# RetamalVictor/marl-range-flocking

Measured on AMD Instinct MI355X. Metric: agent-steps/sec at 256 agents x 4096 envs; 1/2/4/8 MI355X, higher is better.
Workload: dtype f32; 1 GPU; gym_flock_v2 step, 256 agents x 4096 envs per GPU (BASELINE config 3); agents=256, envs_per_gpu=4096, k=4, periodic=True, parallelism=env-shard x1

## Files before the change

marl_range_flocking_amd/csrc/flock_env.hip:

```cpp
#include <hip/hip_runtime.h>

#include <stdint.h>
#include <stdio.h>
#include <stdlib.h>
#include <string.h>

#include "flock_amd.h"
#include "flock_mem.h"

#pragma clang fp contract(off)

namespace {

constexpr int kMem = 4;
constexpr int kSense = 4;
constexpr float kHalfPi = 1.57079637f;
constexpr uint32_t kEmpty = 0xFFFFFFFFu;

thread_local char g_err[256] = "";

int fail(int code, const char* msg) {
    snprintf(g_err, sizeof(g_err), "%s", msg);
    return code;
}
// ... 1747 lines not shown
        FLOCK_CASE(5)
        FLOCK_CASE(6)
        FLOCK_CASE(7)
        FLOCK_CASE(8)
        FLOCK_CASE(9)
        FLOCK_CASE(10)
        FLOCK_CASE(11)
        FLOCK_CASE(12)
        FLOCK_CASE(17)
        default:
            return fail(FLOCK_E_LIMIT, "unsupported k");
    }
#undef FLOCK_CASE
    const hipError_t e = hipGetLastError();
    if (e != hipSuccess) return fail(FLOCK_E_LAUNCH, hipGetErrorString(e));
    return FLOCK_OK;
}

Params base(int E, int N, int k, float box) {
    Params p;
    memset(&p, 0, sizeof(p));
    p.E = E;
    p.N = N;
    p.k = k;
    p.box = box;
    p.clamp = 1;
    return p;
}

}


void flock_sc_diag_no_spec(bool v);
void flock_sc_diag_event_system(bool v);
void flock_sc_diag_free_events(bool v);

extern "C" {

int flock_abi_version(void) { return FLOCK_ABI_VERSION; }

int flock_set_diag(const char* name, int value) {
    if (!name) return fail(FLOCK_E_NULL, "flock_set_diag: NULL name");
    Knobs& k = knobs_mut();
    if (!strcmp(name, "env_launches"))
        k.env_launches = value;
    else if (!strcmp(name, "no_spec"))
        k.no_spec = value != 0;
    else if (!strcmp(name, "no_split"))
        k.no_split = value != 0;
    else if (!strcmp(name, "no_cells"))
        k.no_cells = value != 0;
    else if (!strcmp(name, "pf"))
        k.pf = value;
    else if (!strcmp(name, "rollout_spl") && (value == 2 || value == 4))
        k.rollout_spl = value;
    else if (!strcmp(name, "sc_no_spec"))
        flock_sc_diag_no_spec(value != 0);
    else if (!strcmp(name, "sc_event_system_scope"))
        flock_sc_diag_event_system(value != 0);
    else if (!strcmp(name, "sc_free_events"))
        flock_sc_diag_free_events(value != 0);
    else
        return fail(FLOCK_E_ARG, "flock_set_diag: unknown knob");
    return FLOCK_OK;
}

#ifdef FLOCK_PHASE_PROF
int flock_phase_read(unsigned long long* host) {
    static unsigned long long buf[64 * 32];
    if (hipMemcpyFromSymbol(buf, HIP_SYMBOL(g_phase), sizeof(buf)) != hipSuccess) return 1;
    for (int q = 0; q < 32; ++q) {
        host[q] = 0;
        for (int s = 0; s < 64; ++s) host[q] += buf[s * 32 + q];
    }
    memset(buf, 0, sizeof(buf));
    return hipMemcpyToSymbol(HIP_SYMBOL(g_phase), buf, sizeof(buf)) != hipSuccess;
}
int flock_blk_read(unsigned long long* host) {
    return hipMemcpyFromSymbol(host, HIP_SYMBOL(g_blk), sizeof(g_blk)) != hipSuccess;
}
int flock_blkph_read(unsigned long long* host) {
    return hipMemcpyFromSymbol(host, HIP_SYMBOL(g_blkph), sizeof(g_blkph)) != hipSuccess;
}
#endif

const char* flock_last_error(void) { return g_err; }

}

namespace {
// ... 400 lines not shown
```

marl_range_flocking_amd/csrc/flock_sc.hip:

```cpp
#include <hip/hip_runtime.h>

#include <math.h>
#include <stdint.h>
#include <stdlib.h>

#include "flock_learn.h"
#include "flock_mem.h"
#include "learn_internal.h"

namespace {

using flock_learn_internal::fail;
using flock_learn_internal::launched;

constexpr int kRowsPerBlock = 4;
constexpr int kMaxAct = 4;
constexpr int kMaxIn = 64;
constexpr int kMaxFeat = 1024;
constexpr int kMaxFc1Block = 32768;
constexpr float kLnEps = 1e-5f;

typedef float f32x16 __attribute__((ext_vector_type(16)));

struct CriticOff {
// ... 537 lines not shown
            for (int o = 0; o < kMaxAct; ++o)
                if (o < na) dh = fmaf(aWmu[o * H2 + j], dm[o], dh);
            g2[c] = ag2[j];
        }
        dy2[c] = h2[c] > 0.0f ? dh : 0.0f;
    }
    ln_backward<C>(dy2, xh, g2, rs, H2, dz2);
    store_row<C>(w.AXH2 + ro, xh, H2, lane);
    store_row<C>(w.AH2 + ro, h2, H2, lane);
    store_row<C>(w.ADY2 + ro, dy2, H2, lane);
    store_row<C>(w.ADZ2 + ro, dz2, H2, lane);
    if (lane == 0) w.ARS2[r] = rs;
}

#ifdef FLOCK_SC_PROF
__device__ unsigned long long g_scprof[5][4096][2];
struct ScProf {
    int k;
    unsigned long long t0;
    __device__ explicit ScProf(int kk) : k(kk), t0(__builtin_amdgcn_s_memrealtime()) {}
    __device__ ~ScProf() {
        const int b = blockIdx.x + gridDim.x * blockIdx.y;
        if (b < 4096 && (threadIdx.x & 63) == 0) {
            if (threadIdx.x == 0) g_scprof[k][b][0] = t0;
            atomicMax(&g_scprof[k][b][1], (unsigned long long)__builtin_amdgcn_s_memrealtime());
        }
    }
};
#define SC_PROF(k) ScProf sc_prof_(k)
__device__ unsigned long long g_scmark[4096][8];
#define SC_MARK(MK, i)                                                                           \
    if (MK && threadIdx.x == 0 && blockIdx.x + gridDim.x * blockIdx.y < 4096)                   \
        g_scmark[blockIdx.x + gridDim.x * blockIdx.y][i] = __builtin_amdgcn_s_memrealtime();
#else
#define SC_PROF(k)
#define SC_MARK(MK, i)
#endif
#ifdef FLOCK_SC_PRIO
#define SC_WAVE_PRIO() __builtin_amdgcn_s_setprio(FLOCK_SC_PRIO)
#else
#define SC_WAVE_PRIO()
#endif
constexpr unsigned long long kGateTimeoutTicks = 200000000ull;
__device__ __forceinline__ bool gate_wait(unsigned long long* gate, unsigned long long seq,
                                          unsigned long long* err = nullptr,
                                          unsigned long long ticks = kGateTimeoutTicks) {
    __shared__ int ok;
    if (threadIdx.x == 0) {
        int good = 1;
        if ((long long)(flock_mem::ld_sc1(gate) - seq) < 0) {
            const unsigned long long t0 = __builtin_amdgcn_s_memrealtime();
            while ((long long)(flock_mem::ld_sc1(gate) - seq) < 0) {
                if (__builtin_amdgcn_s_memrealtime() - t0 > ticks) {
                    __hip_atomic_store(err ? err : gate + 1, 1ull, __ATOMIC_RELAXED, __HIP_MEMORY_SCOPE_AGENT);
                    good = 0;
                    break;
                }
                __builtin_amdgcn_s_sleep(2);
            }
        }
        ok = good;
    }
    __syncthreads();
    return ok != 0;
}

__device__ __forceinline__ int xcd_perm(int x, int n) { return (n & 7) == 0 ? (x & 7) * (n >> 3) + (x >> 3) : x; }

template <int C, int HC>
// ... 284 lines not shown
    for (int q = 0; q < 4; ++q) {
        const int m = tm * kT + 8 * wv + 4 * (l >> 5) + q;
        if (m < g.M && n < g.N) g.C[(int64_t)m * g.ldc + n] = g.bias ? out[q] + bias : out[q];
    }
}

template <int AV, int BV, int NF>
__global__ __launch_bounds__(256) void sc_gemm(GemmBatch gb) {
    SC_PROF(1);
    SC_WAVE_PRIO();
    if (gb.done && blockIdx.x == 0 && blockIdx.y == 0 && threadIdx.x == 0) flock_mem::st_sc1(gb.done, gb.done_seq);
    gemm_block<AV, BV, NF>(gb, blockIdx.y, blockIdx.x);
}

struct RedP {
    const float* D;
    const float* X;
    int ldd, ldx, mode, in, n, blk0;
    int64_t off;
};
constexpr int kMaxRed = 12;
#ifndef FLOCK_RED_RB
#define FLOCK_RED_RB 8
#endif
constexpr int kRedElems = 16;
constexpr int kRedGroups = 256 / kRedElems;
constexpr int kMaxRedBlocks = 4096;

struct DzArgs {
    const float *XH, *RS, *PS;
    int F, ntn;
};

__device__ __forceinline__ float red_block(const RedP& rp, int b, int B, const DzArgs& dz, float* part, float* mst,
                                           int& e_out, bool& live_out) {
    const int tid = threadIdx.x;
    const bool dzm = rp.mode == 4 || rp.mode == 5;
    const int el = tid & (kRedElems - 1), q = tid / kRedElems;
    const int e = (b - rp.blk0) * kRedElems + el;
    const bool live = e < rp.n;
    const bool per_in = rp.mode == 2 || rp.mode == 4;
    const int o = per_in ? e / rp.in : e;
    const int i = per_in ? e - o * rp.in : e;
    const bool prod = rp.mode == 1 || rp.mode == 2 || rp.mode == 4;
    constexpr int kRB = FLOCK_RED_RB;
    float dv[kRB], xv[kRB], xh[kRB], rs[kRB];
    auto load = [&](int r0) {
#pragma unroll
        for (int k = 0; k < kRB; ++k) {
            const int r = r0 + kRedGroups * k;
            const bool in = live && r < B;
            dv[k] = in ? rp.D[(int64_t)r * rp.ldd + o] : 0.0f;
            xv[k] = (in && prod) ? rp.X[(int64_t)r * rp.ldx + i] : 0.0f;
            xh[k] = (in && dzm) ? dz.XH[(int64_t)r * dz.F + o] : 0.0f;
            rs[k] = (in && dzm) ? dz.RS[r] : 0.0f;
        }
    };
    load(q);
    if (dzm) {
        for (int r = tid; r < B; r += 256) {
            const float2* ps = reinterpret_cast<const float2*>(dz.PS + (int64_t)r * 2 * dz.ntn);
            float s1 = 0.0f, s2 = 0.0f;
            constexpr int kPB = 16;
            for (int t0 = 0; t0 < dz.ntn; t0 += kPB) {
                float2 v[kPB];
#pragma unroll
                for (int u = 0; u < kPB; ++u)
                    v[u] = t0 + u < dz.ntn ? ps[t0 + u] : make_float2(0.0f, 0.0f);
#pragma unroll
                for (int u = 0; u < kPB; ++u)
                    if (t0 + u < dz.ntn) {
                        s1 += v[u].x;
                        s2 += v[u].y;
                    }
            }
            mst[2 * r] = s1 / (float)dz.F;
            mst[2 * r + 1] = s2 / (float)dz.F;
        }
        __syncthreads();
    }
    float acc = 0.0f;
    for (int r0 = q; r0 < B; r0 += kRedGroups * kRB) {
        if (r0 != q) load(r0);
        if (dzm) {
#pragma unroll
            for (int k = 0; k < kRB; ++k) {
                const int r = min(r0 + kRedGroups * k, B - 1);
                dv[k] = rs[k] * (dv[k] - mst[2 * r] - xh[k] * mst[2 * r + 1]);
            }
        }
#pragma unroll
        for (int k = 0; k < kRB; ++k) acc = prod ? fmaf(dv[k], xv[k], acc) : acc + dv[k];
    }
    part[q * kRedElems + el] = acc;
    __syncthreads();
    float gsum = 0.0f;
    if (q == 0 && live) {
#pragma unroll
        for (int k = 0; k < kRedGroups; ++k) gsum += part[k * kRedElems + el];
    }
    e_out = e;
    live_out = live && q == 0;
    return gsum;
}

struct BwdJob {
    GemmP dh;
    GemmP dw;
    const float *H1, *XH1, *g1;
    float *DY1, *DXH1, *PS1;
    int F, ntn;
    int64_t w2_off;
    int nred, nblk, B;
    RedP red[kMaxRed];
    float* grad;
    int64_t rel;
    int64_t grad_rel;
    const int64_t* agent;
    int64_t agent_v;
    float* loss;
};
__host__ __device__ inline int bwd_blocks(const BwdJob& j) { return j.dh.tiles + j.dw.tiles + j.nblk; }

template <int AVH, int BVH, int AVW, int BVW, int NFH, int NFW>
__device__ __forceinline__ void bwd_body(const BwdJob& j, int bx) {
    extern __shared__ float4 smem4[];
// ... 15 lines not shown
            const int m = tm * kT + 8 * wv + 4 * (l >> 5) + q;
            const bool ok = m < g.M && nok;
            hv[q] = ok ? j.H1[(int64_t)m * j.F + n] : 0.0f;
            xv[q] = ok ? j.XH1[(int64_t)m * j.F + n] : 0.0f;
        }
        float out[4];
        gemm_tile<AVH, BVH, NFH>(g, g.B + relB, tm, tn, smem, out);
        float s1[4], s2[4];
#pragma unroll
        for (int q = 0; q < 4; ++q) {
            const int m = tm * kT + 8 * wv + 4 * (l >> 5) + q;
            const bool ok = m < g.M && nok;
            const float dy = hv[q] > 0.0f ? out[q] : 0.0f;
            const float dxh = dy * gam;
            if (ok) {
                j.DY1[(int64_t)m * j.F + n] = dy;
                j.DXH1[(int64_t)m * j.F + n] = dxh;
            }
            s1[q] = ok ? dxh : 0.0f;
            s2[q] = ok ? dxh * xv[q] : 0.0f;
        }
#pragma unroll
        for (int off = 16; off >= 1; off >>= 1)
#pragma unroll
            for (int q = 0; q < 4; ++q) {
                s1[q] += __shfl_xor(s1[q], off);
                s2[q] += __shfl_xor(s2[q], off);
            }
        if ((l & 31) == 0) {
#pragma unroll
            for (int q = 0; q < 4; ++q) {
                const int m = tm * kT + 8 * wv + 4 * (l >> 5) + q;
                if (m < g.M) {
                    j.PS1[((int64_t)m * j.ntn + tn) * 2] = s1[q];
                    j.PS1[((int64_t)m * j.ntn + tn) * 2 + 1] = s2[q];
                }
            }
        }
    } else if (bx < j.dh.tiles + j.dw.tiles) {
        const GemmP& g = j.dw;
        const int t = bx - j.dh.tiles;
        const int tm = t / g.tiles_n, tn = t - tm * g.tiles_n;
        float out[4];
        gemm_tile<AVW, BVW, NFW>(g, g.B, tm, tn, smem, out);
        const int nn = tn * kT + (l & 31);
#pragma unroll
        for (int q = 0; q < 4; ++q) {
            const int mm = tm * kT + 8 * wv + 4 * (l >> 5) + q;
            if (mm < g.M && nn < g.N) j.grad[gbase + j.w2_off + (int64_t)mm * g.ldc + nn] = out[q];
        }
    } else {
        const int b = bx - j.dh.tiles - j.dw.tiles;
        int q0 = 0;
        for (int q = 1; q < j.nred; ++q)
            if (b >= j.red[q].blk0) q0 = q;
        const RedP& rp = j.red[q0];
        int e;
        bool wr;
        const DzArgs none{nullptr, nullptr, nullptr, 0, 0};
        const float gsum = red_block(rp, b, j.B, none, smem, nullptr, e, wr);
        if (wr) {
            if (rp.mode == 3)
                *j.loss = gsum * (1.0f / (float)j.B);
            else
                j.grad[gbase + rp.off + e] = gsum;
        }
    }
}

struct Bwd2 {
    BwdJob j0, j1;
    int nb0;
    int n0;
};
template <int AVH, int BVH, int AVW, int BVW, int NFH, int NFW>
__global__ __launch_bounds__(256) void sc_bwd(Bwd2 bb) {
    SC_PROF(3);
    SC_WAVE_PRIO();
    if ((int)blockIdx.x < bb.nb0) {
        if ((int)blockIdx.x < bb.n0) bwd_body<AVH, BVH, AVW, BVW, NFH, NFW>(bb.j0, blockIdx.x);
    } else {
        bwd_body<AVH, BVH, AVW, BVW, NFH, NFW>(bb.j1, blockIdx.x - bb.nb0);
    }
}

struct GradAdam {
    int nred, nblk, B, do_adam;
    RedP red[kMaxRed];
    DzArgs dz;
    int64_t adam_lo, adam_n;
    int adam_blocks;
    float *p, *grad, *m, *v;
    int64_t rel;
    int64_t grad_rel;
    const float* grad_scale;
    const int64_t* agent;
    int64_t agent_v;
    int64_t* step;
    unsigned* counter;
    float lr, b1, b2, eps;
    float* target;
    float* self_soft;
    int64_t self_n;
    int soft_rate, soft_blocks;
    float tau, one_minus_tau;
    float* p_copy;
    const int64_t* soft_count;
};
__host__ __device__ inline int late_blocks(const GradAdam& ga) { return ga.nblk + ga.adam_blocks + ga.soft_blocks; }

struct AdamState {
    float p, m, v, t;
};
__device__ __forceinline__ AdamState adam_load(const GradAdam& ga, int64_t i) {
    return {ga.p[i], ga.m[i], ga.v[i], ga.target ? ga.target[i] : 0.0f};
}
__device__ __forceinline__ void adam_store(const GradAdam& ga, int64_t i, AdamState s, float gi, float neg_step,
                                           float bc2s, bool soft) {
    const float w1 = (float)(1.0 - (double)ga.b1), omb2 = (float)(1.0 - (double)ga.b2);
    float mi = s.m;
    mi = (w1 < 0.5f) ? mi + w1 * (gi - mi) : gi - (gi - mi) * (1.0f - w1);
    float vi = s.v * ga.b2;
    vi = vi + (omb2 * gi) * gi;
    const float denom = __builtin_sqrtf(vi) / bc2s + ga.eps;
    const float pn = s.p + (neg_step * mi) / denom;
    if (ga.p_copy) {
        ga.p_copy[i] = pn;
        ga.p[i] = soft ? ga.tau * pn + ga.one_minus_tau * pn : pn;
    } else {
        ga.p[i] = pn;
    }
    ga.m[i] = mi;
    ga.v[i] = vi;
    if (soft && ga.target) ga.target[i] = ga.tau * pn + ga.one_minus_tau * s.t;
}

__device__ __forceinline__ void grad_adam_body(const GradAdam& ga, int bx, int nb) {
    extern __shared__ float4 smem4[];
    float* smem = reinterpret_cast<float*>(smem4);
    __shared__ float sh[2];
    __shared__ int sh_soft;
    const int tid = threadIdx.x;
    const int64_t agent = ga.rel ? agent_at(ga.agent, ga.agent_v) : 0;
    const int64_t base = ga.rel * agent, gbase = ga.grad_rel * agent;
    if (tid == 0) {
        const int64_t step0 = ga.do_adam ? ga.step[agent] : 0;
        const int64_t count = ga.soft_count ? ga.soft_count[agent_at(ga.agent, ga.agent_v)] : step0;
        sh_soft = ga.do_adam && ga.soft_rate > 0 && (count % ga.soft_rate) == 0;
        if (ga.do_adam) {
            const double st = (double)(step0 + 1);
            sh[0] = (float)(-(double)ga.lr / (1.0 - pow((double)ga.b1, st)));
            sh[1] = (float)sqrt(1.0 - pow((double)ga.b2, st));
        }
    }
    const int adam0 = ga.nblk, soft0 = ga.nblk + ga.adam_blocks;
    if (bx >= soft0) {
        __syncthreads();
        if (sh_soft && ga.self_soft) {
            const int64_t b0 = (int64_t)(bx - soft0) * 1024;
#pragma unroll
            for (int q = 0; q < 4; ++q) {
                const int64_t e = b0 + q * 256 + tid;
                if (e < ga.self_n) {
                    const float c = ga.self_soft[e];
                    ga.self_soft[e] = ga.tau * c + ga.one_minus_tau * c;
                }
            }
        }
    } else if (bx >= adam0) {
        const int64_t e0 = ga.adam_lo + (int64_t)(bx - adam0) * 1024, end = ga.adam_lo + ga.adam_n;
        AdamState st[4];
        float gi[4];
        const float gs = ga.grad_scale ? *ga.grad_scale : 1.0f;
#pragma unroll
        for (int q = 0; q < 4; ++q) {
            const int64_t e = e0 + q * 256 + tid;
            st[q] = e < end ? adam_load(ga, base + e) : AdamState{0.f, 0.f, 0.f, 0.f};
            gi[q] = e < end ? ga.grad[gbase + e] : 0.0f;
        }
        __syncthreads();
#pragma unroll
        for (int q = 0; q < 4; ++q) {
            const int64_t e = e0 + q * 256 + tid;
            if (e < end) adam_store(ga, base + e, st[q], ga.grad_scale ? gi[q] * gs : gi[q], sh[0], sh[1], sh_soft != 0);
        }
    } else {
        const int b = bx;
        int q0 = 0;
        for (int q = 1; q < ga.nred; ++q)
            if (b >= ga.red[q].blk0) q0 = q;
        const RedP& rp = ga.red[q0];
        const int e1 = (b - rp.blk0) * kRedElems + (tid & (kRedElems - 1));
        const bool ad = tid / kRedElems == 0 && e1 < rp.n && rp.mode != 3 && ga.do_adam;
        const AdamState st = ad ? adam_load(ga, base + rp.off + e1) : AdamState{0.f, 0.f, 0.f, 0.f};
        int e;
        bool wr;
        const float gsum = red_block(rp, b, ga.B, ga.dz, smem, smem + 256, e, wr);
        if (wr) {
            ga.grad[gbase + rp.off + e] = gsum;
            if (ga.do_adam) adam_store(ga, base + rp.off + e, st, gsum, sh[0], sh[1], sh_soft != 0);
        }
    }
    if (ga.do_adam && tid == 0) {
        const unsigned prev = atomicAdd(ga.counter, 1u);
        if (prev == (unsigned)nb - 1u) {
            ga.step[agent] += 1;
            *ga.counter = 0u;
        }
    }
}

struct GradAdam2 {
    GradAdam j0, j1;
    int nb0;
};
__global__ __launch_bounds__(256) void sc_grad_adam(GradAdam2 gg) {
    SC_PROF(4);
    SC_WAVE_PRIO();
    if ((int)blockIdx.x < gg.nb0)
        grad_adam_body(gg.j0, blockIdx.x, gg.nb0);
    else
        grad_adam_body(gg.j1, blockIdx.x - gg.nb0, gridDim.x - gg.nb0);
}

int balanced_kc(int K, int kcmax) {
    const int n = (K + kcmax - 1) / kcmax;
    const int kc = ((K + n - 1) / n + 7) & ~7;
    return kc < kcmax ? kc : kcmax;
}
int nf_of(int kc) { return kc <= 128 ? 4 : kc <= 224 ? 7 : kc <= 320 ? 10 : 16; }

GemmP gemm_p(const float* A, const float* B, float* C, const float* bias, int M, int N, int K, int sam, int sak,
             int sbk, int sbn, int ldc, int64_t relB, const int64_t* agent = nullptr) {
    GemmP g;
// ... 46 lines not shown
        case 10: return launch_gemm_v<AV, BV, 10>(st, gb, grid, lds);
        default: return launch_gemm_v<AV, BV, 16>(st, gb, grid, lds);
    }
}

int launch_gemm(hipStream_t st, const GemmBatch& gb) {
    int K = 0, kc = 8, tiles = 0, var = gemm_variant(gb.p[0]);
    for (int i = 0; i < gb.n; ++i) {
        K = gb.p[i].K > K ? gb.p[i].K : K;
        const int c = gemm_kc(gb.p[i].K, gb.p[i].kchunk);
        kc = c > kc ? c : kc;
        tiles = gb.p[i].tiles > tiles ? gb.p[i].tiles : tiles;
        if (gemm_variant(gb.p[i]) != var) var = 3;
    }
    const dim3 grid(tiles, gb.n);
    const size_t lds = gemm_lds_bytes(kc, kc);
    const int nf = nf_of(kc);
    switch (var) {
        case 0: return launch_gemm_nf<0, 0>(st, gb, grid, lds, nf);
        case 1: return launch_gemm_nf<0, 1>(st, gb, grid, lds, nf);
        case 2: return launch_gemm_nf<1, 1>(st, gb, grid, lds, nf);
        default: return launch_gemm_v<2, 2, 16>(st, gb, grid, lds);
    }
}

template <typename J>
void add_red(J& ga, const float* D, int ldd, const float* X, int ldx, int mode, int in, int n, int64_t off) {
    const int j = ga.nred++;
    RedP& r = ga.red[j];
    r.D = D; r.X = X; r.ldd = ldd; r.ldx = ldx; r.mode = mode; r.in = in; r.n = n; r.off = off;
    r.blk0 = ga.nblk;
    ga.nblk += (n + kRedElems - 1) / kRedElems;
}
size_t red_lds(int B) { return (size_t)(256 + 2 * B) * sizeof(float); }
size_t bwd_lds(const BwdJob& j) {
    const size_t a = gemm_lds_bytes(j.dh.K, j.dh.kchunk), b = gemm_lds_bytes(j.dw.K, j.dw.kchunk);
    const size_t r = 256 * sizeof(float);
    return a > b ? (a > r ? a : r) : (b > r ? b : r);
}

template <int AVH, int BVH, int AVW, int BVW, int NFH, int NFW>
int launch_bwd_v(hipStream_t st, const Bwd2& bb, dim3 grid, size_t lds) {
    if (int rc = allow_lds(sc_bwd<AVH, BVH, AVW, BVW, NFH, NFW>, lds)) return rc;
    hipLaunchKernelGGL((sc_bwd<AVH, BVH, AVW, BVW, NFH, NFW>), grid, dim3(256), lds, st, bb);
    return launched();
}

int check(const FlockScUpdate* u) {
    if (!u) return fail(-3, "flock_sc: NULL argument");
    if (u->B < 1 || u->in_dim < 1 || u->n_actions < 1 || u->fc1 < 1 || u->fc2 < 1)
        return fail(-5, "flock_sc: sizes must be >= 1");
    if (u->in_dim > kMaxIn || u->n_actions > kMaxAct || u->fc1 > kMaxFeat || u->fc2 > kMaxFeat ||
        u->fc1 * (u->in_dim + 3) > kMaxFc1Block)
        return fail(-2, "flock_sc: in_dim <= 64, n_actions <= 4, fc1/fc2 <= 1024, fc1 * (in_dim + 3) <= 32768");
    if (!u->idx || !u->agent || !u->ring_state || !u->ring_new_state || !u->ring_action || !u->ring_reward ||
        !u->ring_terminal || !u->critic || !u->critic_grad || !u->actors || !u->actors_grad || !u->actors_target ||
        !u->losses || !u->workspace || !u->counters)
        return fail(-3, "flock_sc: NULL pointer");
    if (u->do_adam && (!u->critic_exp_avg || !u->critic_exp_avg_sq || !u->critic_step || !u->actors_exp_avg ||
                       !u->actors_exp_avg_sq || !u->actor_steps))
        return fail(-3, "flock_sc: NULL optimizer state");
    const ActorOff ao = actor_off(u->in_dim, u->n_actions, u->fc1, u->fc2);
    if (u->actor_stride < ao.total) return fail(-5, "flock_sc: actor_stride smaller than one actor");
    return 0;
}

int chunks(const FlockScUpdate* u) {
// ... 30 lines not shown
    GemmP fwd[3];
    int nfwd;
    BwdJob bw;
    GradAdam ga;
    bool free_dev;
};

void job_common(const FlockScUpdate* u, Job& j) {
    j.B = u->B; j.in = u->in_dim; j.na = u->n_actions; j.H1 = u->fc1; j.H2 = u->fc2;
    ws_layout(j.B, j.in, j.na, j.H1, j.H2, u->workspace, &j.w);
    j.a = row_args(u);
    j.C = chunks(u);
    j.rb = (j.B + kRowsPerBlock - 1) / kRowsPerBlock;
    j.lds1 = fc1_lds(j.in, j.H1);
    j.lds3 = tails_lds(j.na, j.H2);
    j.free_dev = false;
}

void bwd_common(Job& j, const float* W2, int64_t rel_w2, const int64_t* agent, const float* H1, const float* XH1,
                const float* g1, float* DY1, float* DXH1, float* PS1, const float* DZ2, int64_t w2_off, float* grad,
                int64_t rel, float* loss) {
    const int B = j.B, H1n = j.H1, H2 = j.H2;
    BwdJob& bw = j.bw;
    bw.dh = gemm_p(DZ2, W2, nullptr, nullptr, B, H1n, H2, H2, 1, H1n, 1, H1n, rel_w2, agent);
    bw.dw = gemm_p(DZ2, H1, nullptr, nullptr, H2, H1n, B, 1, H2, H1n, 1, H1n, 0);
    bw.dw.kchunk = balanced_kc(B, kGradKC);
    bw.H1 = H1; bw.XH1 = XH1; bw.g1 = g1; bw.DY1 = DY1; bw.DXH1 = DXH1; bw.PS1 = PS1;
    bw.F = H1n; bw.ntn = bw.dh.tiles_n;
    bw.w2_off = w2_off;
    bw.nred = 0; bw.nblk = 0; bw.B = B;
    bw.grad = grad; bw.rel = rel; bw.grad_rel = rel; bw.agent = agent; bw.agent_v = -1; bw.loss = loss;
}

void late_common(Job& j, const FlockScUpdate* u, const float* DXH1, const float* DY1, const float* XH1,
                 const float* RS1, const float* PS1, int64_t W1, int64_t b1, int64_t g1, int64_t be1, int64_t W2,
                 int64_t total) {
    const int in = j.in, H1 = j.H1;
    GradAdam& ga = j.ga;
    ga.nred = 0;
    ga.nblk = 0;
    ga.B = j.B;
    ga.do_adam = u->do_adam;
    add_red(ga, DXH1, H1, j.w.S, in, 4, in, H1 * in, W1);
    add_red(ga, DXH1, H1, nullptr, 0, 5, 1, H1, b1);
    add_red(ga, DY1, H1, XH1, H1, 1, 1, H1, g1);
    add_red(ga, DY1, H1, nullptr, 0, 0, 1, H1, be1);
    ga.dz = DzArgs{XH1, RS1, PS1, H1, j.bw.ntn};
    ga.adam_lo = W2;
    ga.adam_n = total - W2;
    ga.adam_blocks = u->do_adam ? (int)((ga.adam_n + 1023) / 1024) : 0;
    ga.lr = 0.0f;
    ga.grad_scale = nullptr;
    ga.b1 = u->beta1; ga.b2 = u->beta2; ga.eps = u->eps;
    ga.tau = u->tau;
    ga.one_minus_tau = (float)(1.0 - (double)u->tau);
}

void critic_job(const FlockScUpdate* u, Job& j) {
    job_common(u, j);
    const int B = j.B, in = j.in, na = j.na, H1 = j.H1, H2 = j.H2;
    const Ws& w = j.w;
    const CriticOff co = critic_off(in, na, H1, H2);
    const ActorOff ao = actor_off(in, na, H1, H2);
    j.fwd[0] = gemm_p(w.TH1, u->actors_target + ao.W2, w.Z2, u->actors_target + ao.b2, B, H2, H1, H1, 1, 1, H1, H2,
                      u->actor_stride, u->agent);
    j.fwd[1] = gemm_p(w.NH1, u->critic + co.W2, w.Z2 + (int64_t)B * H2, u->critic + co.b2, B, H2, H1, H1, 1, 1, H1,
                      H2, 0);
    j.fwd[2] = gemm_p(w.H1, u->critic + co.W2, w.Z2 + 2 * (int64_t)B * H2, u->critic + co.b2, B, H2, H1, H1, 1, 1,
                      H1, H2, 0);
    j.nfwd = 3;
    BwdJob& bw = j.bw;
    bwd_common(j, u->critic + co.W2, 0, u->agent, w.H1, w.XH1, u->critic + co.g1, w.DY1, w.DXH1, w.PS1, w.DZ2, co.W2,
               u->critic_grad, 0, u->losses + 1);
    add_red(bw, w.DZ2, H2, nullptr, 0, 0, 1, H2, co.b2);
    add_red(bw, w.DY2, H2, w.XH2, H2, 1, 1, H2, co.g2);
    add_red(bw, w.DY2, H2, nullptr, 0, 0, 1, H2, co.be2);
    add_red(bw, w.DZA, H2, w.A, na, 2, na, H2 * na, co.Wa);
    add_red(bw, w.DZA, H2, nullptr, 0, 0, 1, H2, co.ba);
    add_red(bw, w.DQ, 1, w.HQ, H2, 2, H2, H2, co.Wq);
// ... 227 lines not shown
    }
    for (int c = 0; c < n_actions; ++c) st(dst.action + (int64_t)r * n_actions + c, src.action[row * n_actions + c]);
    const float rw = src.reward[row], te = src.terminal[row];
    st(dst.reward + r, rw);
    st(dst.terminal + r, te);
}

__global__ __launch_bounds__(64) void sc_prep_snapshot(int B, int64_t rows, uint64_t seed, uint64_t counter,
                                                        int64_t* idx_out, int64_t* agent_out, int64_t agent,
                                                        int in_dim, int n_actions, FlockScRows src,
                                                        FlockScRows dst, int vec) {
    const int r = blockIdx.x * 64 + threadIdx.x;
    if (r == 0) *agent_out = agent;
    if (r < B) snapshot_row<false>(rows, seed, counter, idx_out, in_dim, n_actions, src, dst, vec, r);
}

__global__ __launch_bounds__(256) void sc_prep_snapshot_gate(int B, int64_t rows, uint64_t seed, uint64_t counter,
                                                             int64_t* agent_out, int64_t agent, int in_dim,
                                                             int n_actions, FlockScRows src, FlockScRows dst, int vec,
                                                             unsigned long long* gate, unsigned long long seq,
                                                             unsigned long long reuse, unsigned long long ticks) {
    if (reuse && !gate_wait(gate + 2, reuse, gate + 1, ticks)) return;
    if (threadIdx.x == 0) flock_mem::st_sc1(agent_out, agent);
    for (int r = threadIdx.x; r < B; r += 256)
        snapshot_row<true>(rows, seed, counter, nullptr, in_dim, n_actions, src, dst, vec, r);
    flock_mem::wait_vmem();
    __syncthreads();
    if (threadIdx.x == 0) __hip_atomic_store(gate, seq, __ATOMIC_RELAXED, __HIP_MEMORY_SCOPE_AGENT);
}

}

void flock_sc_diag_no_spec(bool v) { g_sc_no_spec = v; }
void flock_sc_diag_event_system(bool v);

int round_adam(void* stream, const FlockScUpdate* critic_u, const FlockScUpdate* actor_u, const float* grad_scale,
               int64_t agent_c, int64_t agent_a);
extern "C" {

int flock_sc_prep_snapshot(void* stream, int B, int64_t rows, uint64_t seed, uint64_t counter, int64_t* idx_out,
                           int64_t* agent_out, int64_t agent, int in_dim, int n_actions, const FlockScRows* ring,
                           const FlockScRows* staging) {
    if (!agent_out || !ring || !staging) return fail(-3, "flock_sc_prep_snapshot: NULL pointer");
    if (B < 1 || rows < 1 || in_dim < 1 || n_actions < 1)
        return fail(-5, "flock_sc_prep_snapshot: need B, rows, in_dim, n_actions >= 1");
    const FlockScRows* rs[2] = {ring, staging};
    for (const FlockScRows* x : rs)
        if (!x->state || !x->new_state || !x->action || !x->reward || !x->terminal)
            return fail(-3, "flock_sc_prep_snapshot: NULL field pointer");
    int vec = in_dim == 4 && n_actions == 2;
    for (const FlockScRows* x : rs)
        vec = vec && al16(x->state) && al16(x->new_state) && (((uintptr_t)x->action & 7) == 0);
    hipLaunchKernelGGL(sc_prep_snapshot, dim3((B + 63) / 64), dim3(64), 0, (hipStream_t)stream, B, rows, seed,
                       counter, idx_out, agent_out, agent, in_dim, n_actions, *ring, *staging, vec);
    return launched();
}

int flock_sc_prep(void* stream, int B, int64_t rows, uint64_t seed, uint64_t counter, int64_t* idx,
                  int64_t* agent_out, int64_t agent) {
    if (!agent_out) return fail(-3, "flock_sc_prep: NULL agent pointer");
    if (idx && (B < 1 || rows < 1)) return fail(-5, "flock_sc_prep: need B >= 1 and rows >= 1");
    const int blocks = idx ? (B + 255) / 256 : 1;
    hipLaunchKernelGGL(sc_prep, dim3(blocks), dim3(256), 0, (hipStream_t)stream, B, rows, seed, counter, idx,
                       agent_out, agent);
    return launched();
}
// ... 7 lines not shown
int flock_sc_critic_update(void* stream, const FlockScUpdate* u) { return flock_sc_round(stream, u, nullptr); }

int flock_sc_actor_update(void* stream, const FlockScUpdate* u) { return flock_sc_round(stream, nullptr, u); }

int flock_sc_round_adam(void* stream, const FlockScUpdate* critic_u, const FlockScUpdate* actor_u,
                        const float* grad_scale) {
    return round_adam(stream, critic_u, actor_u, grad_scale, -1, -1);
}
}

int round_adam(void* stream, const FlockScUpdate* critic_u, const FlockScUpdate* actor_u, const float* grad_scale,
               int64_t agent_c, int64_t agent_a) {
    if (!critic_u && !actor_u) return fail(-3, "flock_sc_round_adam: NULL argument");
    int rc = 0;
    if (critic_u && (rc = check(critic_u))) return rc;
    if (actor_u && (rc = check(actor_u))) return rc;
    if ((critic_u && !critic_u->do_adam) || (actor_u && !actor_u->do_adam))
        return fail(-5, "flock_sc_round_adam: the updates must have do_adam = 1");
    Job jc, ja;
    GradAdam* js[2] = {nullptr, nullptr};
    int n = 0;
    if (critic_u) {
        critic_job(critic_u, jc);
        js[n++] = &jc.ga;
    }
    if (actor_u) {
        actor_job(actor_u, ja);
        js[n++] = &ja.ga;
    }
    for (int i = 0; i < n; ++i) {
        GradAdam& g = *js[i];
        g.nred = 0;
        g.nblk = 0;
        g.adam_lo = 0;
        g.grad_scale = grad_scale;
    }
    if (critic_u) {
        const CriticOff co = critic_off(critic_u->in_dim, critic_u->n_actions, critic_u->fc1, critic_u->fc2);
        jc.ga.adam_n = co.total;
        jc.ga.adam_blocks = (int)((co.total + 1023) / 1024);
    }
    if (actor_u) {
        const ActorOff ao = actor_off(actor_u->in_dim, actor_u->n_actions, actor_u->fc1, actor_u->fc2);
        ja.ga.adam_n = ao.total;
        ja.ga.adam_blocks = (int)((ao.total + 1023) / 1024);
    }
    if (critic_u) jc.ga.agent_v = agent_c;
    if (actor_u) ja.ga.agent_v = agent_a;
    GradAdam2 gg;
    gg.j0 = *js[0];
    gg.j1 = *js[n - 1];
    gg.nb0 = late_blocks(gg.j0);
    const int nb = gg.nb0 + (n == 2 ? late_blocks(gg.j1) : 0);
    hipLaunchKernelGGL(sc_grad_adam, dim3(nb), dim3(256), 0, (hipStream_t)stream, gg);
    return launched();
}
extern "C" {

int flock_sc_round(void* stream, const FlockScUpdate* critic_u, const FlockScUpdate* actor_u) {
    if (!critic_u && !actor_u) return fail(-3, "flock_sc_round: NULL argument");
    int rc = 0;
    if (critic_u && (rc = check(critic_u))) return rc;
    if (actor_u && (rc = check(actor_u))) return rc;
    Job jc, ja;
    if (critic_u) critic_job(critic_u, jc);
    if (actor_u) actor_job(actor_u, ja);
// ... 411 lines not shown
    for (int i = 0; i < p->n; ++i) {
        p->ug[i].actor_grad_out = actor_grads[i];
        p->uadam[i].actor_grad_out = actor_grads[i];
        actor_job(&p->ug[i], p->jga[i]);
    }
    p->actor_allreduce = allreduce;
    p->actor_ctx = ctx;
    p->split = true;
    return 0;
}

int flock_sc_pipeline_flush(FlockScPipeline* p, void* learner_stream) {
    if (!p) return fail(-3, "flock_sc_pipeline_flush: NULL pipeline");
    hipStream_t ls = (hipStream_t)learner_stream;
    const int q = p->pending;
    if (q >= 0) {
        if (int rc = pipeline_round(p, ls, -1, q, -1, p->pending_agent)) return rc;
        if (int rc = p->gseq[q] ? 0 : emit_free_point(p, ls, q)) return rc;
        p->pending = -1;
    }
    if (p->split && (hipEventRecord(p->actor_joined, p->actor_stream) != hipSuccess ||
                     hipStreamWaitEvent(ls, p->actor_joined, 0) != hipSuccess))
        return fail(-4, "flock_sc_pipeline_flush: stream operation failed");
    return 0;
}

#ifdef FLOCK_SC_PROF
int flock_sc_prof_read(unsigned long long* host) {
    return hipMemcpyFromSymbol(host, HIP_SYMBOL(g_scprof), sizeof(g_scprof)) != hipSuccess;
}
int flock_sc_mark_read(unsigned long long* host) {
    return hipMemcpyFromSymbol(host, HIP_SYMBOL(g_scmark), sizeof(g_scmark)) != hipSuccess;
}
#endif

int flock_sc_pipeline_check(FlockScPipeline* p) {
    if (!p) return fail(-3, "flock_sc_pipeline_check: NULL pipeline");
    if (!p->gate) return 0;
    unsigned long long flag = 0;
    if (hipMemcpy(&flag, p->gate + 1, sizeof(flag), hipMemcpyDeviceToHost) != hipSuccess)
        return fail(-4, "flock_sc_pipeline_check: copy failed");
    return flag ? fail(-6, "flock_sc_pipeline: a learn() round gave up waiting for its minibatch snapshot (device gate "
                           "timeout); its results are invalid")
                : 0;
}

int flock_sc_pipeline_gated(const FlockScPipeline* p) { return p && p->gate_on ? 1 : 0; }

}
void flock_sc_diag_event_system(bool v) { g_sc_event_system = v; }
void flock_sc_diag_free_events(bool v) { g_sc_free_events = v; }
extern "C" {

void* flock_sc_pipeline_comm_stream(const FlockScPipeline* p) { return p ? (void*)p->comm_stream : nullptr; }

int64_t flock_sc_pipeline_gated_learns(const FlockScPipeline* p) { return p ? p->gated_learns : 0; }

void flock_sc_pipeline_destroy(FlockScPipeline* p) {
    if (!p) return;
    if (p->gate) (void)hipFree(p->gate);
    if (p->actor_stream) (void)hipStreamDestroy(p->actor_stream);
    if (p->actor_joined) (void)hipEventDestroy(p->actor_joined);
    if (p->comm_stream) (void)hipStreamDestroy(p->comm_stream);
    if (p->bwd_done) (void)hipEventDestroy(p->bwd_done);
    if (p->ar_done) (void)hipEventDestroy(p->ar_done);
    if (p->mark_ev) (void)hipEventDestroy(p->mark_ev);
// ... 14 lines not shown
```

Before: 14.61 billion agent-steps/s.

## Fuse first-layer weight/bias/LN grad reductions into one block pass

```diff
diff --git a/marl_range_flocking_amd/csrc/flock_env.hip b/marl_range_flocking_amd/csrc/flock_env.hip
--- a/marl_range_flocking_amd/csrc/flock_env.hip
+++ b/marl_range_flocking_amd/csrc/flock_env.hip
@@ -1803,6 +1803,7 @@
 
 
 void flock_sc_diag_no_spec(bool v);
+void flock_sc_diag_red_legacy(bool v);
 void flock_sc_diag_event_system(bool v);
 void flock_sc_diag_free_events(bool v);
 
@@ -1827,6 +1828,8 @@
         k.rollout_spl = value;
     else if (!strcmp(name, "sc_no_spec"))
         flock_sc_diag_no_spec(value != 0);
+    else if (!strcmp(name, "sc_red_legacy"))
+        flock_sc_diag_red_legacy(value != 0);
     else if (!strcmp(name, "sc_event_system_scope"))
         flock_sc_diag_event_system(value != 0);
     else if (!strcmp(name, "sc_free_events"))
diff --git a/marl_range_flocking_amd/csrc/flock_sc.hip b/marl_range_flocking_amd/csrc/flock_sc.hip
--- a/marl_range_flocking_amd/csrc/flock_sc.hip
+++ b/marl_range_flocking_amd/csrc/flock_sc.hip
@@ -593,9 +593,13 @@
 #define SC_MARK(MK, i)                                                                           \
     if (MK && threadIdx.x == 0 && blockIdx.x + gridDim.x * blockIdx.y < 4096)                   \
         g_scmark[blockIdx.x + gridDim.x * blockIdx.y][i] = __builtin_amdgcn_s_memrealtime();
+__device__ unsigned long long g_sclate[4096][4];
+#define SC_LMARK(MK, i) \
+    if (MK && threadIdx.x == 0 && blockIdx.x < 4096) g_sclate[blockIdx.x][i] = __builtin_amdgcn_s_memrealtime();
 #else
 #define SC_PROF(k)
 #define SC_MARK(MK, i)
+#define SC_LMARK(MK, i)
 #endif
 #ifdef FLOCK_SC_PRIO
 #define SC_WAVE_PRIO() __builtin_amdgcn_s_setprio(FLOCK_SC_PRIO)
@@ -946,6 +950,33 @@
     int F, ntn;
 };
 
+__device__ __forceinline__ float ln1_dz(float rs, float dxh, float xh, float m1, float m2) {
+    return rs * (dxh - m1 - xh * m2);
+}
+
+__device__ __forceinline__ void ln1_row_stats(const DzArgs& dz, int B, float* mst) {
+    const float2* ps = reinterpret_cast<const float2*>(dz.PS);
+    for (int r = threadIdx.x; r < B; r += 256) {
+        float s1 = 0.0f, s2 = 0.0f;
+        constexpr int kPB = 16;
+        for (int t0 = 0; t0 < dz.ntn; t0 += kPB) {
+            float2 v[kPB];
+#pragma unroll
+            for (int u = 0; u < kPB; ++u)
+                v[u] = t0 + u < dz.ntn ? ps[(int64_t)(t0 + u) * B + r] : make_float2(0.0f, 0.0f);
+#pragma unroll
+            for (int u = 0; u < kPB; ++u)
+                if (t0 + u < dz.ntn) {
+                    s1 += v[u].x;
+                    s2 += v[u].y;
+                }
+        }
+        mst[2 * r] = s1 / (float)dz.F;
+        mst[2 * r + 1] = s2 / (float)dz.F;
+    }
+}
+
+template <int MK = 0>
 __device__ __forceinline__ float red_block(const RedP& rp, int b, int B, const DzArgs& dz, float* part, float* mst,
                                            int& e_out, bool& live_out) {
     const int tid = threadIdx.x;
@@ -970,29 +1001,13 @@
             rs[k] = (in && dzm) ? dz.RS[r] : 0.0f;
         }
     };
+    SC_LMARK(MK, 0)
     load(q);
     if (dzm) {
-        for (int r = tid; r < B; r += 256) {
-            const float2* ps = reinterpret_cast<const float2*>(dz.PS + (int64_t)r * 2 * dz.ntn);
-            float s1 = 0.0f, s2 = 0.0f;
-            constexpr int kPB = 16;
-            for (int t0 = 0; t0 < dz.ntn; t0 += kPB) {
-                float2 v[kPB];
-#pragma unroll
-                for (int u = 0; u < kPB; ++u)
-                    v[u] = t0 + u < dz.ntn ? ps[t0 + u] : make_float2(0.0f, 0.0f);
-#pragma unroll
-                for (int u = 0; u < kPB; ++u)
-                    if (t0 + u < dz.ntn) {
-                        s1 += v[u].x;
-                        s2 += v[u].y;
-                    }
-            }
-            mst[2 * r] = s1 / (float)dz.F;
-            mst[2 * r + 1] = s2 / (float)dz.F;
-        }
+        ln1_row_stats(dz, B, mst);
         __syncthreads();
     }
+    SC_LMARK(MK, 1)
     float acc = 0.0f;
     for (int r0 = q; r0 < B; r0 += kRedGroups * kRB) {
         if (r0 != q) load(r0);
@@ -1000,12 +1015,13 @@
 #pragma unroll
             for (int k = 0; k < kRB; ++k) {
                 const int r = min(r0 + kRedGroups * k, B - 1);
-                dv[k] = rs[k] * (dv[k] - mst[2 * r] - xh[k] * mst[2 * r + 1]);
+                dv[k] = ln1_dz(rs[k], dv[k], xh[k], mst[2 * r], mst[2 * r + 1]);
             }
         }
 #pragma unroll
         for (int k = 0; k < kRB; ++k) acc = prod ? fmaf(dv[k], xv[k], acc) : acc + dv[k];
     }
+    SC_LMARK(MK, 2)
     part[q * kRedElems + el] = acc;
     __syncthreads();
     float gsum = 0.0f;
@@ -1087,8 +1103,8 @@
             for (int q = 0; q < 4; ++q) {
                 const int m = tm * kT + 8 * wv + 4 * (l >> 5) + q;
                 if (m < g.M) {
-                    j.PS1[((int64_t)m * j.ntn + tn) * 2] = s1[q];
-                    j.PS1[((int64_t)m * j.ntn + tn) * 2 + 1] = s2[q];
+                    j.PS1[((int64_t)tn * j.B + m) * 2] = s1[q];
+                    j.PS1[((int64_t)tn * j.B + m) * 2 + 1] = s2[q];
                 }
             }
         }
@@ -1143,6 +1159,9 @@
     int nred, nblk, B, do_adam;
     RedP red[kMaxRed];
     DzArgs dz;
+    int fused_in;
+    const float *fDXH, *fDY, *fS;
+    int64_t fW1, fb1, fg1, fbe1;
     int64_t adam_lo, adam_n;
     int adam_blocks;
     float *p, *grad, *m, *v;
@@ -1190,6 +1209,76 @@
     if (soft && ga.target) ga.target[i] = ga.tau * pn + ga.one_minus_tau * s.t;
 }
 
+constexpr int kFusedPitch = 256 + 8;
+template <int IN>
+__device__ __forceinline__ void fused_block(const GradAdam& ga, int b, int64_t base, int64_t gbase, float* smem,
+                                            const float* sh, const int& sh_soft) {
+    static_assert(IN == 4, "one 16-B load of the row's inputs");
+    constexpr int kNV = IN + 3, kOut = kRedElems * kNV, kRB = FLOCK_RED_RB;
+    const int tid = threadIdx.x, B = ga.B, F = ga.dz.F;
+    const int el = tid & (kRedElems - 1), q = tid / kRedElems;
+    const int o = b * kRedElems + el;
+    const bool live = o < F;
+    float* mst = smem + kNV * kFusedPitch;
+    SC_LMARK(1, 0)
+    const int v = tid < kRedElems * IN ? tid % IN : IN + (tid - kRedElems * IN) / kRedElems;
+    const int c = tid < kRedElems * IN ? tid / IN : (tid - kRedElems * IN) % kRedElems;
+    const int oc = b * kRedElems + c;
+    const bool wr = tid < kOut && oc < F;
+    const int64_t poff = v < IN ? ga.fW1 + (int64_t)oc * IN + v : (v == IN ? ga.fb1 : v == IN + 1 ? ga.fg1 : ga.fbe1) + oc;
+    const AdamState st = (wr && ga.do_adam) ? adam_load(ga, base + poff) : AdamState{0.f, 0.f, 0.f, 0.f};
+    float dxh[kRB], dy[kRB], xh[kRB], rs[kRB];
+    float4 sv[kRB];
+    auto load = [&](int r0) {
+#pragma unroll
+        for (int k = 0; k < kRB; ++k) {
+            const int r = r0 + kRedGroups * k;
+            const bool in = live && r < B;
+            dxh[k] = in ? ga.fDXH[(int64_t)r * F + o] : 0.0f;
+            dy[k] = in ? ga.fDY[(int64_t)r * F + o] : 0.0f;
+            xh[k] = in ? ga.dz.XH[(int64_t)r * F + o] : 0.0f;
+            rs[k] = in ? ga.dz.RS[r] : 0.0f;
+            sv[k] = in ? *reinterpret_cast<const float4*>(ga.fS + (int64_t)r * IN) : make_float4(0.f, 0.f, 0.f, 0.f);
+        }
+    };
+    load(q);
+    ln1_row_stats(ga.dz, B, mst);
+    __syncthreads();
+    SC_LMARK(1, 1)
+    float aw[IN] = {0.0f, 0.0f, 0.0f, 0.0f}, ab = 0.0f, ag = 0.0f, abe = 0.0f;
+    for (int r0 = q; r0 < B; r0 += kRedGroups * kRB) {
+        if (r0 != q) load(r0);
+#pragma unroll
+        for (int k = 0; k < kRB; ++k) {
+            const int r = min(r0 + kRedGroups * k, B - 1);
+            const float dz = ln1_dz(rs[k], dxh[k], xh[k], mst[2 * r], mst[2 * r + 1]);
+            aw[0] = fmaf(dz, sv[k].x, aw[0]);
+            aw[1] = fmaf(dz, sv[k].y, aw[1]);
+            aw[2] = fmaf(dz, sv[k].z, aw[2]);
+            aw[3] = fmaf(dz, sv[k].w, aw[3]);
+            ab = ab + dz;
+            ag = fmaf(dy[k], xh[k], ag);
+            abe = abe + dy[k];
+        }
+    }
+    SC_LMARK(1, 2)
+    const int slot = q * kRedElems + el;
+#pragma unroll
+    for (int i = 0; i < IN; ++i) smem[i * kFusedPitch + slot] = aw[i];
+    smem[IN * kFusedPitch + slot] = ab;
+    smem[(IN + 1) * kFusedPitch + slot] = ag;
+    smem[(IN + 2) * kFusedPitch + slot] = abe;
+    __syncthreads();
+    if (wr) {
+        float gsum = 0.0f;
+#pragma unroll
+        for (int k = 0; k < kRedGroups; ++k) gsum += smem[v * kFusedPitch + k * kRedElems + c];
+        ga.grad[gbase + poff] = gsum;
+        if (ga.do_adam) adam_store(ga, base + poff, st, gsum, sh[0], sh[1], sh_soft != 0);
+    }
+    SC_LMARK(1, 3)
+}
+
 __device__ __forceinline__ void grad_adam_body(const GradAdam& ga, int bx, int nb) {
     extern __shared__ float4 smem4[];
     float* smem = reinterpret_cast<float*>(smem4);
@@ -1198,17 +1287,22 @@
     const int tid = threadIdx.x;
     const int64_t agent = ga.rel ? agent_at(ga.agent, ga.agent_v) : 0;
     const int64_t base = ga.rel * agent, gbase = ga.grad_rel * agent;
-    if (tid == 0) {
+    const int adam0 = ga.nblk, soft0 = ga.nblk + ga.adam_blocks;
+    if (tid < 2) {
         const int64_t step0 = ga.do_adam ? ga.step[agent] : 0;
-        const int64_t count = ga.soft_count ? ga.soft_count[agent_at(ga.agent, ga.agent_v)] : step0;
-        sh_soft = ga.do_adam && ga.soft_rate > 0 && (count % ga.soft_rate) == 0;
+        if (tid == 0) {
+            const int64_t count = ga.soft_count ? ga.soft_count[agent_at(ga.agent, ga.agent_v)] : step0;
+            sh_soft = ga.do_adam && ga.soft_rate > 0 && (count % ga.soft_rate) == 0;
+        }
         if (ga.do_adam) {
             const double st = (double)(step0 + 1);
-            sh[0] = (float)(-(double)ga.lr / (1.0 - pow((double)ga.b1, st)));
-            sh[1] = (float)sqrt(1.0 - pow((double)ga.b2, st));
-        }
-    }
-    const int adam0 = ga.nblk, soft0 = ga.nblk + ga.adam_blocks;
+            const double pw = pow(tid == 0 ? (double)ga.b1 : (double)ga.b2, st);
+            if (tid == 0)
+                sh[0] = (float)(-(double)ga.lr / (1.0 - pw));
+            else
+                sh[1] = (float)sqrt(1.0 - pw);
+        }
+    }
     if (bx >= soft0) {
         __syncthreads();
         if (sh_soft && ga.self_soft) {
@@ -1239,6 +1333,8 @@
             const int64_t e = e0 + q * 256 + tid;
             if (e < end) adam_store(ga, base + e, st[q], ga.grad_scale ? gi[q] * gs : gi[q], sh[0], sh[1], sh_soft != 0);
         }
+    } else if (ga.fused_in == 4) {
+        fused_block<4>(ga, bx, base, gbase, smem, sh, sh_soft);
     } else {
         const int b = bx;
         int q0 = 0;
@@ -1250,11 +1346,12 @@
         const AdamState st = ad ? adam_load(ga, base + rp.off + e1) : AdamState{0.f, 0.f, 0.f, 0.f};
         int e;
         bool wr;
-        const float gsum = red_block(rp, b, ga.B, ga.dz, smem, smem + 256, e, wr);
+        const float gsum = red_block<1>(rp, b, ga.B, ga.dz, smem, smem + 256, e, wr);
         if (wr) {
             ga.grad[gbase + rp.off + e] = gsum;
             if (ga.do_adam) adam_store(ga, base + rp.off + e, st, gsum, sh[0], sh[1], sh_soft != 0);
         }
+        SC_LMARK(1, 3)
     }
     if (ga.do_adam && tid == 0) {
         const unsigned prev = atomicAdd(ga.counter, 1u);
@@ -1367,7 +1464,7 @@
     r.blk0 = ga.nblk;
     ga.nblk += (n + kRedElems - 1) / kRedElems;
 }
-size_t red_lds(int B) { return (size_t)(256 + 2 * B) * sizeof(float); }
+size_t red_lds(int B) { return (size_t)(7 * kFusedPitch + 2 * B) * sizeof(float); }
 size_t bwd_lds(const BwdJob& j) {
     const size_t a = gemm_lds_bytes(j.dh.K, j.dh.kchunk), b = gemm_lds_bytes(j.dw.K, j.dw.kchunk);
     const size_t r = 256 * sizeof(float);
@@ -1464,6 +1561,8 @@
     bw.grad = grad; bw.rel = rel; bw.grad_rel = rel; bw.agent = agent; bw.agent_v = -1; bw.loss = loss;
 }
 
+bool g_sc_red_legacy = false;
+
 void late_common(Job& j, const FlockScUpdate* u, const float* DXH1, const float* DY1, const float* XH1,
                  const float* RS1, const float* PS1, int64_t W1, int64_t b1, int64_t g1, int64_t be1, int64_t W2,
                  int64_t total) {
@@ -1473,10 +1572,17 @@
     ga.nblk = 0;
     ga.B = j.B;
     ga.do_adam = u->do_adam;
-    add_red(ga, DXH1, H1, j.w.S, in, 4, in, H1 * in, W1);
-    add_red(ga, DXH1, H1, nullptr, 0, 5, 1, H1, b1);
-    add_red(ga, DY1, H1, XH1, H1, 1, 1, H1, g1);
-    add_red(ga, DY1, H1, nullptr, 0, 0, 1, H1, be1);
+    ga.fused_in = (!g_sc_red_legacy && in == 4) ? in : 0;
+    ga.fDXH = DXH1; ga.fDY = DY1; ga.fS = j.w.S;
+    ga.fW1 = W1; ga.fb1 = b1; ga.fg1 = g1; ga.fbe1 = be1;
+    if (ga.fused_in) {
+        ga.nblk = (H1 + kRedElems - 1) / kRedElems;
+    } else {
+        add_red(ga, DXH1, H1, j.w.S, in, 4, in, H1 * in, W1);
+        add_red(ga, DXH1, H1, nullptr, 0, 5, 1, H1, b1);
+        add_red(ga, DY1, H1, XH1, H1, 1, 1, H1, g1);
+        add_red(ga, DY1, H1, nullptr, 0, 0, 1, H1, be1);
+    }
     ga.dz = DzArgs{XH1, RS1, PS1, H1, j.bw.ntn};
     ga.adam_lo = W2;
     ga.adam_n = total - W2;
@@ -1770,6 +1876,7 @@
 }
 
 void flock_sc_diag_no_spec(bool v) { g_sc_no_spec = v; }
+void flock_sc_diag_red_legacy(bool v) { g_sc_red_legacy = v; }
 void flock_sc_diag_event_system(bool v);
 
 int round_adam(void* stream, const FlockScUpdate* critic_u, const FlockScUpdate* actor_u, const float* grad_scale,
@@ -1843,6 +1950,7 @@
         GradAdam& g = *js[i];
         g.nred = 0;
         g.nblk = 0;
+        g.fused_in = 0;
         g.adam_lo = 0;
         g.grad_scale = grad_scale;
     }
@@ -2320,6 +2428,9 @@
 int flock_sc_mark_read(unsigned long long* host) {
     return hipMemcpyFromSymbol(host, HIP_SYMBOL(g_scmark), sizeof(g_scmark)) != hipSuccess;
 }
+int flock_sc_late_mark_read(unsigned long long* host) {
+    return hipMemcpyFromSymbol(host, HIP_SYMBOL(g_sclate), sizeof(g_sclate)) != hipSuccess;
+}
 #endif
 
 int flock_sc_pipeline_check(FlockScPipeline* p) {
```

After: 14.86 billion agent-steps/s, median of 6. +1.7%, better.
